# yewsiang/Transferable3D

Hardware: AMD Instinct MI355X
Metric: frustums/sec fwd+bwd (higher is better)
Workload: dtype f32

## Files before the change

transferable3d_amd/csrc/pointmlp.hip:

```cpp
#include "common.h"
#include "poolbwd_dev.h"
#include "rider_dev.h"

#include <cstdlib>
#include <mutex>
#include <type_traits>
#include <utility>
#include <unordered_map>

namespace {

constexpr int BK = 32;
constexpr int MIN_WAVES_PER_EU = 2;
constexpr int LDR = BK + 4;
constexpr int NT = 256;

__device__ __forceinline__ float4 f4zero() { return make_float4(0.f, 0.f, 0.f, 0.f); }

__device__ __forceinline__ unsigned keep_bits32(const float* __restrict__ rowmask, int base) {
  float4 m[8];
#pragma unroll
  for (int q = 0; q < 8; ++q) m[q] = *reinterpret_cast<const float4*>(rowmask + base + (q >> 2) * 32 + (q & 3) * 8);
  unsigned bits = 0u;
#pragma unroll
// ... 1285 lines not shown
    c.sh = *reinterpret_cast<const float4*>(reinterpret_cast<const char*>(shp + ucol) + lbytes);
    return c;
  }
  static constexpr bool HAS_CTAB = true;
  __device__ __forceinline__ int ctab_floats() const { return 2 * K; }
  __device__ __forceinline__ void ctab_fill(float* tab, int tid, int nthreads) const {
    const float* scp = s.scale != nullptr ? s.scale : t3d_ident_scale;
    const float* shp = s.scale != nullptr ? s.shift : t3d_ident_shift;
    for (int i = tid * 4; i < K; i += nthreads * 4) {
      *reinterpret_cast<float4*>(tab + i) = *reinterpret_cast<const float4*>(scp + i);
      *reinterpret_cast<float4*>(tab + K + i) = *reinterpret_cast<const float4*>(shp + i);
    }
  }
  __device__ __forceinline__ Coef ctab_coef(const float* tab, int col) const {
    Coef c;
    c.sc = *reinterpret_cast<const float4*>(tab + col);
    c.sh = *reinterpret_cast<const float4*>(tab + K + col);
    return c;
  }
  __device__ __forceinline__ Coef fetch_coef(int col) const {
    Coef c;
    c.sc = make_float4(1.f, 1.f, 1.f, 1.f);
    c.sh = f4zero();
    if (s.scale != nullptr) {
      c.sc = *reinterpret_cast<const float4*>(s.scale + col);
      c.sh = *reinterpret_cast<const float4*>(s.shift + col);
    }
    return c;
  }
  __device__ __forceinline__ Raw fetch(int row, int col) const {
    Raw r;
    r.x = *reinterpret_cast<const float4*>(s.x + (size_t)row * s.ldx + s.coff + col);
    return r;
  }
  __device__ __forceinline__ float4 xform(const Raw& r, const Coef& c, int, int) const {
    const float floor_ = s.relu ? 0.f : -INFINITY;
    return make_float4(fmaxf(fmaf(r.x.x, c.sc.x, c.sh.x), floor_), fmaxf(fmaf(r.x.y, c.sc.y, c.sh.y), floor_),
                       fmaxf(fmaf(r.x.z, c.sc.z, c.sh.z), floor_), fmaxf(fmaf(r.x.w, c.sc.w, c.sh.w), floor_));
  }
};

struct PathX3 {
  typedef float T;
  template <bool HAS_SUB, class XT> using Act = std::conditional_t<HAS_SUB, ActLoader<true>, ActLoaderE>;
  template <bool POOLED> using Dy = DyLoader<POOLED>;
  typedef WLoaderT<float> WL;
  typedef WLoaderT<float, true> WLX;
  static constexpr bool BF16 = false;
  static constexpr bool X3 = true;
  static constexpr int RED = BKX;
  template <int DIM, bool TYPE_R, class L, int PF, bool IS_A = false> using Stg = StagerX3<DIM, TYPE_R, L>;
};
template <class WL, bool FWD = true, class Args>
__device__ __forceinline__ WL make_wloader(const Args& p) {
  if constexpr (IsFrag<WL>::value) return WL{reinterpret_cast<const bf16_t*>(p.w_x3), (long)p.w_x3_stride, FWD ? p.N / 32 : p.K / 32};
  else return WL{p.w, p.N, p.K, p.N};
}
struct PathX3P : PathX3 {
  typedef WLoaderX3F WL;
  typedef WLoaderX3F WLX;
  template <int DIM, bool TYPE_R, class L, int PF, bool IS_A = false>
  using Stg = std::conditional_t<IsFrag<L>::value, StagerX3F<DIM, TYPE_R, L>, StagerX3<DIM, TYPE_R, L>>;
};
struct PathX3W : PathX3 {
  static constexpr int WAVES = 8;
  template <int DIM, bool TYPE_R, class L, int PF, bool IS_A = false> using Stg = StagerX3<DIM, TYPE_R, L, 2 * NT>;
};
struct PathX3WP : PathX3W {
  typedef WLoaderX3F WL;
  typedef WLoaderX3F WLX;
  template <int DIM, bool TYPE_R, class L, int PF, bool IS_A = false>
  using Stg = std::conditional_t<IsFrag<L>::value, StagerX3F<DIM, TYPE_R, L>, StagerX3<DIM, TYPE_R, L, 2 * NT>>;
};
template <class PR, class = void> struct WavesOf { static constexpr int value = 4; };
template <class PR> struct WavesOf<PR, typename std::enable_if<(PR::WAVES > 0)>::type> { static constexpr int value = PR::WAVES; };
template <class PR, int TM, int TN, class SA, class SB, class LA, class LB, bool AR, int DIMA, bool BR, int DIMB, bool SYM = false>
__device__ __forceinline__ void run_mainloop(SA& sa, SB& sb, const LA& la, const LB& lb, float* smem, int red_begin, int red_end,
                                             int a0, int b0, f32x16 (&acc)[TM][TN], int tid) {
  if constexpr (PR::X3) gemm_mainloop_x3<SYM, TM, TN, SA, SB, LA, LB, AR, DIMA, BR, DIMB>(sa, sb, la, lb, smem, red_begin, red_end, a0, b0, acc, tid);
  else if constexpr (PR::BF16) gemm_mainloop_h<TM, TN, SA, SB, LA, LB, AR, DIMA, BR, DIMB>(sa, sb, la, lb, smem, red_begin, red_end, a0, b0, acc, tid);
  else gemm_mainloop<TM, TN, SA, SB, LA, LB, AR, DIMA, BR, DIMB>(sa, sb, la, lb, smem, red_begin, red_end, a0, b0, acc, tid);
}

template <int BN, bool HAS_SUB, class PR = PathF32, class XT = float>
__device__ __forceinline__ void fwd_body(const t3d_pointmlp_fwd_args& p, float* smem, const int bid, const int nblk) {
  constexpr int BM = 128, TM = 2;
  constexpr int WN = WavesOf<PR>::value / 2, WCOLS = BN / WN, TN = WCOLS / 32;
  static_assert(TN == 1 || TN == 2, "a wave owns 32 or 64 columns");
  using LA = typename PR::template Act<HAS_SUB, XT>;
  using YT = typename PR::T;
  using WL = std::conditional_t<LA::EXACT, typename PR::WLX, typename PR::WL>;
  using SA = typename PR::template Stg<BM, true, LA, (PR::BF16 && BN == 128 && !Elem<XT>::BF16) ? 0 : 1, true>;
  using SB = typename PR::template Stg<BN, false, WL, 1>;

  const int tid = (int)threadIdx.x, lane = tid & 63, wid = tid >> 6;
  const int wm = wid / WN, wn = wid % WN;
  const int tiles_n = p.N / BN;
  const int lin = xcd_remap(bid, nblk);
  const int tile_m = lin / tiles_n, tile_n = lin % tiles_n;
  const int row0 = tile_m * BM, col0 = tile_n * BN;
  T3D_TRACE_MARK(0);

  LA la{p.a, p.K, p.rows_per_frustum};
  WL lb = make_wloader<WL>(p);
  SA sa; SB sb;
  sa.init(la, row0, tid);
  sb.init(lb, col0, tid);

  float addv[TN], addr[TN];
  {
    const int l31_ = lane & 31, b_ = row0 / p.rows_per_frustum;
#pragma unroll
    for (int tn = 0; tn < TN; ++tn) {
      const int col = col0 + wn * WCOLS + tn * 32 + l31_;
      addv[tn] = p.bias ? p.bias[col] : 0.f;
      addr[tn] = p.rowbias ? p.rowbias[(size_t)b_ * p.N + col] : 0.f;
    }
  }
  const bool has_rowbias = p.rowbias != nullptr;
  f32x16 acc[TM][TN];
  zero_acc<TM, TN>(acc);
  const int kred = (p.K + PR::RED - 1) / PR::RED * PR::RED;
  run_mainloop<PR, TM, TN, SA, SB, LA, WL, true, BM, false, BN>(sa, sb, la, lb, smem, 0, kred, wm * 64,
                                                                     wn * WCOLS, acc, tid);
  T3D_TRACE_MARK(1);

  const int l31 = lane & 31, h = lane >> 5;
  const int b = row0 / p.rows_per_frustum;
  const bool pool = p.pmax != nullptr;
  const bool store_y = p.y != nullptr;
  float* red = smem;
  constexpr int YLD = BN + 8;
  bf16_t* ytile = reinterpret_cast<bf16_t*>(smem + 12 * BN);
  float csum[TN], csq[TN], cmax[TN], cmin[TN];
  int amax[TN], amin[TN];
  unsigned keepbits = 0xffffffffu;
  if (pool && p.rowmask) {
    static_assert(TM == 2, "keep_bits32 covers two 32-row blocks");
    keepbits = keep_bits32(p.rowmask, row0 + wm * 64 + 4 * h);
  }
  const int rin_base = row0 - b * p.rows_per_frustum + wm * 64 + 4 * h;
  const unsigned n4 = (unsigned)p.N * 4u;
  char* const yb = reinterpret_cast<char*>(p.y);
  auto epi = [&](auto sy_tag, auto pl_tag) {
    constexpr bool SY = decltype(sy_tag)::value, PL = decltype(pl_tag)::value;
#pragma unroll
    for (int tn = 0; tn < TN; ++tn) {
      const int col = col0 + wn * WCOLS + tn * 32 + l31;
      const float add = has_rowbias ? addv[tn] + addr[tn] : addv[tn];
      float s = 0.f, ss = 0.f, mx = -INFINITY, mn = INFINITY;
      int ax = -1, an = -1;
      unsigned boff0 = ((unsigned)(row0 + wm * 64 + 4 * h) * (unsigned)p.N + (unsigned)col) * 4u;
      asm volatile("" : "+v"(boff0));
#pragma unroll
      for (int tm = 0; tm < TM; ++tm) {
#pragma unroll
        for (int r = 0; r < 16; ++r) {
          const float v = SY ? Elem<YT>::rnd(acc[tm][tn][r] + add) : acc[tm][tn][r] + add;
          if constexpr (SY) {
            if constexpr (Elem<YT>::BF16) {
              ytile[(wm * 64 + 4 * h + tm * 32 + (r & 3) + 8 * (r >> 2)) * YLD + wn * WCOLS + tn * 32 + l31] = (bf16_t)v;
            } else {
              *reinterpret_cast<float*>(yb + (boff0 + (unsigned)(tm * 32 + (r & 3) + 8 * (r >> 2)) * n4)) = v;
            }
          }
          s += v;
          ss = fmaf(v, v, ss);
          if constexpr (PL) {
            const bool keep = (keepbits >> (tm * 16 + r)) & 1u;
            const int rin = rin_base + tm * 32 + (r & 3) + 8 * (r >> 2);
            const bool up = keep & (v > mx), dn = keep & (v < mn);
            mx = up ? v : mx;
            ax = up ? rin : ax;
            mn = dn ? v : mn;
            an = dn ? rin : an;
          }
        }
      }
      s += __shfl_xor(s, 32, 64);
      ss += __shfl_xor(ss, 32, 64);
      if constexpr (PL) {
        const float omx = __shfl_xor(mx, 32, 64), omn = __shfl_xor(mn, 32, 64);
        const int oax = __shfl_xor(ax, 32, 64), oan = __shfl_xor(an, 32, 64);
        if (oax >= 0 && (omx > mx || ax < 0 || (omx == mx && oax < ax))) { mx = omx; ax = oax; }
        if (oan >= 0 && (omn < mn || an < 0 || (omn == mn && oan < an))) { mn = omn; an = oan; }
      }
      csum[tn] = s; csq[tn] = ss; cmax[tn] = mx; cmin[tn] = mn; amax[tn] = ax; amin[tn] = an;
    }
  };
  if (store_y) { if (pool) epi(std::true_type{}, std::true_type{}); else epi(std::true_type{}, std::false_type{}); }
  else { if (pool) epi(std::false_type{}, std::true_type{}); else epi(std::false_type{}, std::false_type{}); }
  __syncthreads();
  if (h == 0) {
#pragma unroll
    for (int tn = 0; tn < TN; ++tn) {
      const int c = wn * WCOLS + tn * 32 + l31;
      red[(0 * 2 + wm) * BN + c] = csum[tn];
      red[(1 * 2 + wm) * BN + c] = csq[tn];
      if (pool) {
        red[(2 * 2 + wm) * BN + c] = cmax[tn];
        red[(3 * 2 + wm) * BN + c] = cmin[tn];
        reinterpret_cast<int*>(red)[(4 * 2 + wm) * BN + c] = amax[tn];
        reinterpret_cast<int*>(red)[(5 * 2 + wm) * BN + c] = amin[tn];
      }
    }
  }
  __syncthreads();
  if (tid < BN) {
    const int c = tid;
    const size_t o = (size_t)tile_m * p.N + col0 + c;
    p.psum[o] = red[(0 * 2 + 0) * BN + c] + red[(0 * 2 + 1) * BN + c];
    p.psumsq[o] = red[(1 * 2 + 0) * BN + c] + red[(1 * 2 + 1) * BN + c];
    if (pool) {
      float mx = red[(2 * 2 + 0) * BN + c], mn = red[(3 * 2 + 0) * BN + c];
      int ax = reinterpret_cast<int*>(red)[(4 * 2 + 0) * BN + c], an = reinterpret_cast<int*>(red)[(5 * 2 + 0) * BN + c];
      const float mx1 = red[(2 * 2 + 1) * BN + c], mn1 = red[(3 * 2 + 1) * BN + c];
      const int ax1 = reinterpret_cast<int*>(red)[(4 * 2 + 1) * BN + c], an1 = reinterpret_cast<int*>(red)[(5 * 2 + 1) * BN + c];
      if (ax1 >= 0 && (ax < 0 || mx1 > mx)) { mx = mx1; ax = ax1; }
      if (an1 >= 0 && (an < 0 || mn1 < mn)) { mn = mn1; an = an1; }
      p.pmax[o] = mx; p.pmin[o] = mn; p.pamax[o] = ax; p.pamin[o] = an;
    }
  }
  if (store_y) {
    if constexpr (Elem<YT>::BF16) {
      constexpr int CPR = BN / 8;
      bf16_t* yg = reinterpret_cast<bf16_t*>(p.y);
#pragma unroll
      for (int i = 0; i < 128 * CPR / NT; ++i) {
        const int c = tid + NT * i, row = c / CPR, ch = c % CPR;
        const bf16x8 v = *reinterpret_cast<const bf16x8*>(ytile + row * YLD + ch * 8);
        *reinterpret_cast<bf16x8*>(yg + (size_t)(row0 + row) * p.N + col0 + ch * 8) = v;
      }
    }
  }
  T3D_TRACE_MARK(2);
}

template <int BN, bool HAS_SUB, class PR = PathF32, class XT = float>
__global__ __launch_bounds__(NT, MIN_WAVES_PER_EU) void k_pointmlp_fwd(const t3d_pointmlp_fwd_args p) {
  extern __shared__ __attribute__((aligned(16))) float smem[];
  fwd_body<BN, HAS_SUB, PR, XT>(p, smem, blockIdx.x, gridDim.x);
}

template <int BN, class PR>
__global__ __launch_bounds__(2 * NT) void k_pointmlp_fwd_w8(const t3d_pointmlp_fwd_args p, const int n_tiles) {
  extern __shared__ __attribute__((aligned(16))) float smem[];
  for (int b = blockIdx.x; b < n_tiles; b += gridDim.x) {
    int bb = b;
    asm volatile("" : "+s"(bb));
    fwd_body<BN, false, PR, float>(p, smem, bb, n_tiles);
    __syncthreads();
  }
}
template <int BN, class PR>
__global__ __launch_bounds__(2 * NT) void k_pointmlp_fwd_w8_r(const t3d_pointmlp_fwd_args p, const t3d_rider_set r, const int n_tiles) {
  extern __shared__ __attribute__((aligned(16))) float smem[];
  if ((int)blockIdx.x < r.n_wg) {
    if (threadIdx.x >= NT) return;
    run_riders(r, smem);
    return;
  }
  for (int b = blockIdx.x - r.n_wg; b < n_tiles; b += gridDim.x - r.n_wg) {
    int bb = b;
    asm volatile("" : "+s"(bb));
    fwd_body<BN, false, PR, float>(p, smem, bb, n_tiles);
    __syncthreads();
  }
}

template <int BN, bool HAS_SUB, class PR = PathF32>
__global__ __launch_bounds__(NT, MIN_WAVES_PER_EU) void k_pointmlp_fwd_r(const t3d_pointmlp_fwd_args p, const t3d_rider_set r) {
  extern __shared__ __attribute__((aligned(16))) float smem[];
  if ((int)blockIdx.x < r.n_wg) { run_riders(r, smem); return; }
  fwd_body<BN, HAS_SUB, PR, float>(p, smem, blockIdx.x - r.n_wg, gridDim.x - r.n_wg);
}

template <int BN, int KT>
__global__ __launch_bounds__(NT, MIN_WAVES_PER_EU) void k_pointmlp_fwd_res(const t3d_pointmlp_fwd_args p) {
  constexpr int TM = 2, TN = BN / 64, ST = BKH / 16;
  using LA = ActLoaderT<false, bf16_t>;
  using WL = WLoaderT<bf16_t, true>;
  using SA = StagerHSel<128, true, LA, KT>;
  using SB = StagerHSel<BN, false, WL, 1>;
  constexpr int A_ELEMS = SA::LDS_ELEMS, B_ELEMS = SB::LDS_ELEMS;
  static_assert((size_t)2 * B_ELEMS * 2 >= (size_t)12 * BN * 4 + (size_t)128 * (BN + 8) * 2, "the epilogue scratch aliases the weight ring");
  extern __shared__ __attribute__((aligned(16))) float smem[];
  bf16_t* panel = reinterpret_cast<bf16_t*>(smem);
  bf16_t* bst = panel + KT * A_ELEMS;

  const int tid0 = threadIdx.x;
  int tid = tid0, lane = tid & 63, wid = tid >> 6;
  int wm = wid >> 1, wn = wid & 1, l31 = lane & 31, h = lane >> 5;
  const bool pool = p.pmax != nullptr, store_y = p.y != nullptr;
  const int tiles_m = p.M / 128, G = gridDim.x;
  LA la{p.a, p.K, p.rows_per_frustum};
  SA sa;
  constexpr bool PREF = KT <= 2;
  auto fetch_panel = [&](int t_m) {
    sa.init(la, t_m * 128, tid);
    sa.template fetch_raw<0>(la, 0, tid);
    if constexpr (KT > 1) sa.template fetch_raw<1>(la, BKH, tid);
    if constexpr (KT > 2) { sa.template fetch_raw<2>(la, 2 * BKH, tid); sa.template fetch_raw<3>(la, 3 * BKH, tid); }
  };
  auto fetch_panel_coefs = [&]() {
    sa.template fetch_coefs<0>(la, 0, tid);
    if constexpr (KT > 1) sa.template fetch_coefs<1>(la, BKH, tid);
    if constexpr (KT > 2) { sa.template fetch_coefs<2>(la, 2 * BKH, tid); sa.template fetch_coefs<3>(la, 3 * BKH, tid); }
  };
  WL lb{p.w, p.N, p.K, p.N};
  SB sb;
  const int n_tiles = p.N / BN;
  float addv[TN], addr[TN];
  const bool has_rowbias = p.rowbias != nullptr;
  auto fetch_w0 = [&](int c0, int bb) {
    sb.init(lb, c0, tid);
    sb.template fetch<0>(lb, 0, tid);
#pragma unroll
    for (int tn = 0; tn < TN; ++tn) {
      const int col = c0 + wn * (BN / 2) + tn * 32 + l31;
      addv[tn] = p.bias ? p.bias[col] : 0.f;
      addr[tn] = has_rowbias ? p.rowbias[(size_t)bb * p.N + col] : 0.f;
    }
  };
  int tile_m = xcd_remap(blockIdx.x, G);
  T3D_TRACE_MARK8(0);
  if constexpr (PREF) { fetch_panel(tile_m); fetch_panel_coefs(); }
  fetch_w0(0, (tile_m * 128) / p.rows_per_frustum);
#pragma unroll 1
 for (; tile_m < tiles_m; tile_m += G) {
  const bool tr_first = tile_m < G;
  tid = tid0;
  asm volatile("" : "+v"(tid));
  lane = tid & 63; wid = tid >> 6; wm = wid >> 1; wn = wid & 1; l31 = lane & 31; h = lane >> 5;
  const int row0 = tile_m * 128;
  const int b = row0 / p.rows_per_frustum;
  if constexpr (!PREF) { fetch_panel(tile_m); fetch_panel_coefs(); }
  sa.template store<0>(la, panel, tid);
  if constexpr (KT > 1) sa.template store<1>(la, panel + A_ELEMS, tid);
  if constexpr (KT > 2) { sa.template store<2>(la, panel + 2 * A_ELEMS, tid); sa.template store<3>(la, panel + 3 * A_ELEMS, tid); }
  if (tr_first) T3D_TRACE_MARK8(1);
  unsigned keepbits = 0xffffffffu;
  if (pool && p.rowmask) {
    static_assert(TM == 2, "keep_bits32 covers two 32-row blocks");
    keepbits = keep_bits32(p.rowmask, row0 + wm * 64 + 4 * h);
  }
  const int rin_base = row0 - b * p.rows_per_frustum + wm * 64 + 4 * h;
  float* red = reinterpret_cast<float*>(bst);
  constexpr int YLD = BN + 8, CPR = BN / 8;
  bf16_t* ytile = reinterpret_cast<bf16_t*>(red + 12 * BN);
// ... 1911 lines not shown
                                                       const t3d_x3_frag_entry* __restrict__ tab, int n) {
  split_x3_frag_body(params, pf, pd, stride, tab, n, (int)blockIdx.x);
}

template <int N>
__global__ __launch_bounds__(NT) void k_step_head(const t3d_pointmlp_fwd_args p, const int n_fwd, const float* __restrict__ params,
                                                  bf16_t* __restrict__ pf, bf16_t* __restrict__ pd, const long stride,
                                                  const t3d_x3_frag_entry* __restrict__ tab, const int n, const int n_split, float* hyper,
                                                  const t3d_schedule sched) {
  __shared__ float red[2][NT / (N / 8)][N];
  const int b = blockIdx.x;
  if (b < n_fwd) pointmlp_fwd_tinyk_body<N, float>(p, red, b);
  else if (b < n_fwd + n_split) split_x3_frag_body(params, pf, pd, stride, tab, n, b - n_fwd);
  else if (threadIdx.x < 64) schedule_step_body(hyper, sched, threadIdx.x);
}
}
int t3d_x3_step_head(const t3d_pointmlp_fwd_args* a, const float* params, void* pf, void* pd, int64_t stride, const t3d_x3_frag_entry* tab, int n,
                     int n_blocks, float* hyper, const t3d_schedule* sched, hipStream_t s) {
  static_assert(NT == 256, "the three roles of k_step_head are 256-thread workgroups");
  const int n_fwd = a->M / 128;
  const dim3 grid(n_fwd + n_blocks + 1);
  if (a->N == 64) T3D_LAUNCH(k_step_head<64>, grid, dim3(NT), 0, s, *a, n_fwd, params, static_cast<bf16_t*>(pf), static_cast<bf16_t*>(pd), (long)stride, tab, n, n_blocks, hyper, *sched);
  else T3D_LAUNCH(k_step_head<128>, grid, dim3(NT), 0, s, *a, n_fwd, params, static_cast<bf16_t*>(pf), static_cast<bf16_t*>(pd), (long)stride, tab, n, n_blocks, hyper, *sched);
  T3D_CHECK_LAUNCH();
  return T3D_OK;
}
int t3d_x3_split_frag(const float* params, void* pf, void* pd, int64_t stride, const t3d_x3_frag_entry* tab, int n, int n_blocks, hipStream_t s) {
  T3D_LAUNCH(k_split_x3_frag, dim3(n_blocks), dim3(256), 0, s, params, static_cast<bf16_t*>(pf), static_cast<bf16_t*>(pd), (long)stride, tab, n);
  T3D_CHECK_LAUNCH();
  return T3D_OK;
}
int t3d_x3_split(const float* src, void* planes, int64_t n, int64_t plane_stride, hipStream_t s) {
  long blocks = (n + 1023) / 1024;
  if (blocks > 2048) blocks = 2048;
  T3D_LAUNCH(k_split_x3, dim3((unsigned)blocks), dim3(256), 0, s, src, static_cast<bf16_t*>(planes), (long)n, (long)plane_stride);
  T3D_CHECK_LAUNCH();
  return T3D_OK;
}

int t3d_x3_dgrad(const t3d_pointmlp_dgrad_args* a, bool wide, hipStream_t s) {
  const int tiles_m = a->M / 128;
  if (a->w_x3 && (a->K % 32 != 0 || a->N % 16 != 0 || a->w_x3_stride < (int64_t)a->K * a->N)) return T3D_ERR_SHAPE;
  if (a->w_x3 && a->N <= X3_CTAB_MAX_CH) {
    if (wide) launch_lds(k_pointmlp_dgrad<128, false, PathX3P>, dim3(tiles_m * (a->K / 128)), lds_dgrad_x3(128), s, *a);
    else launch_lds(k_pointmlp_dgrad<64, false, PathX3P>, dim3(tiles_m * (a->K / 64)), lds_dgrad_x3(64), s, *a);
  } else if (wide) launch_lds(k_pointmlp_dgrad<128, false, PathX3>, dim3(tiles_m * (a->K / 128)), lds_dgrad_x3(128), s, *a);
  else launch_lds(k_pointmlp_dgrad<64, false, PathX3>, dim3(tiles_m * (a->K / 64)), lds_dgrad_x3(64), s, *a);
  T3D_CHECK_LAUNCH();
  return T3D_OK;
}

int t3d_x3_wgrad(const t3d_pointmlp_wgrad_args* a, int tk, int tn, int n_blocks, hipStream_t s) {
  const dim3 grid(n_blocks);
#define T3D_WGX(TK, TN_) launch_lds(k_pointmlp_wgrad<TK, TN_, false, false, PathX3, float>, grid, lds_wgrad_x3(TK, TN_), s, *a)
  if (tk == 128 && tn == 128) T3D_WGX(128, 128);
  else if (tk == 128) T3D_WGX(128, 64);
  else if (tn == 128) T3D_WGX(64, 128);
  else T3D_WGX(64, 64);
#undef T3D_WGX
  T3D_CHECK_LAUNCH();
  return T3D_OK;
}

int t3d_x3_gram(const t3d_pointmlp_gram_args* a, int tk, int n_blocks, hipStream_t s) {
  if (tk != 64) return T3D_ERR_ARG;
  launch_lds(k_pointmlp_gram<64, 64, PathX3>, dim3(n_blocks), lds_wgrad_x3(64, 64), s, *a);
  T3D_CHECK_LAUNCH();
  return T3D_OK;
}

int t3d_x3_dgrad_gram(const t3d_pointmlp_dgrad_gram_args* a, bool wide, hipStream_t s) {
  const int tiles_m = a->M / 128;
  if (wide) launch_lds(k_pointmlp_dgrad_gram<128, PathX3>, dim3(tiles_m * (a->K / 128)), lds_fwd_x3(128), s, *a);
  else launch_lds(k_pointmlp_dgrad_gram<64, PathX3>, dim3(tiles_m * (a->K / 64)), lds_fwd_x3(64), s, *a);
  T3D_CHECK_LAUNCH();
  return T3D_OK;
}

int t3d_x3_fwd(const t3d_pointmlp_fwd_args* a, const t3d_rider_set* r, hipStream_t s) {
  const int tiles_m = a->M / 128, nr = r ? r->n_wg : 0;
  const bool pre = a->w_x3 != nullptr && a->K <= X3_CTAB_MAX_CH;
  if (pre && (a->N % 32 != 0 || a->K % 16 != 0 || a->w_x3_stride < (int64_t)a->K * a->N)) return T3D_ERR_SHAPE;
  const int w8 = []() { const char* e_ = getenv("T3D_X3_W8"); return e_ ? atoi(e_) : 1; }();
  if (w8 && a->N % 256 == 0 && (w8 == 2 || (long)tiles_m * (a->N / 256) >= 512)) {
    const int n_tiles = tiles_m * (a->N / 256);
    const dim3 grid((n_tiles > T3D_FAIR_CUS ? T3D_FAIR_CUS : n_tiles) + nr);
    const size_t lds = lds_with(lds_fwd_x3(256), r);
    if (r && pre) {
      auto kern = k_pointmlp_fwd_w8_r<256, PathX3WP>;
      allow_lds(reinterpret_cast<const void*>(kern), lds);
      T3D_LAUNCH(kern, grid, dim3(2 * NT), lds, s, *a, *r, n_tiles);
    } else if (r) {
      auto kern = k_pointmlp_fwd_w8_r<256, PathX3W>;
      allow_lds(reinterpret_cast<const void*>(kern), lds);
      T3D_LAUNCH(kern, grid, dim3(2 * NT), lds, s, *a, *r, n_tiles);
    } else if (pre) {
      auto kern = k_pointmlp_fwd_w8<256, PathX3WP>;
      allow_lds(reinterpret_cast<const void*>(kern), lds);
      T3D_LAUNCH(kern, grid, dim3(2 * NT), lds, s, *a, n_tiles);
    } else {
      auto kern = k_pointmlp_fwd_w8<256, PathX3W>;
      allow_lds(reinterpret_cast<const void*>(kern), lds);
      T3D_LAUNCH(kern, grid, dim3(2 * NT), lds, s, *a, n_tiles);
    }
    T3D_CHECK_LAUNCH();
    return T3D_OK;
  }
  if (a->N % 128 == 0 && (long)tiles_m * (a->N / 128) >= 512) {
    const dim3 grid(tiles_m * (a->N / 128) + nr);
    if (r && pre) launch_lds_r(k_pointmlp_fwd_r<128, false, PathX3P>, grid, lds_with(lds_fwd_x3(128), r), s, *a, *r);
    else if (r) launch_lds_r(k_pointmlp_fwd_r<128, false, PathX3>, grid, lds_with(lds_fwd_x3(128), r), s, *a, *r);
    else if (pre) launch_lds(k_pointmlp_fwd<128, false, PathX3P, float>, grid, lds_fwd_x3(128), s, *a);
    else launch_lds(k_pointmlp_fwd<128, false, PathX3, float>, grid, lds_fwd_x3(128), s, *a);
  } else {
    const dim3 grid(tiles_m * (a->N / 64) + nr);
    if (r && pre) launch_lds_r(k_pointmlp_fwd_r<64, false, PathX3P>, grid, lds_with(lds_fwd_x3(64), r), s, *a, *r);
    else if (r) launch_lds_r(k_pointmlp_fwd_r<64, false, PathX3>, grid, lds_with(lds_fwd_x3(64), r), s, *a, *r);
    else if (pre) launch_lds(k_pointmlp_fwd<64, false, PathX3P, float>, grid, lds_fwd_x3(64), s, *a);
    else launch_lds(k_pointmlp_fwd<64, false, PathX3, float>, grid, lds_fwd_x3(64), s, *a);
  }
  T3D_CHECK_LAUNCH();
  return T3D_OK;
}

int t3d_x3_bwd(const t3d_pointmlp_dgrad_args* d, const t3d_pointmlp_wgrad_args* w, const t3d_rider_set* r, int tk, int tn, bool wide,
               int n_w, int n_d, hipStream_t s) {
  if (d->w_x3 && (d->K % 32 != 0 || d->N % 16 != 0 || d->w_x3_stride < (int64_t)d->K * d->N)) return T3D_ERR_SHAPE;
  const dim3 grid(n_w + n_d + (r ? r->n_wg : 0));
#define T3D_BWDX_P(DBN, TK, TN_, PR_)                                                             \
  do {                                                                                             \
    const size_t lds = lds_max(lds_dgrad_x3(DBN), lds_wgrad_x3(TK, TN_));                          \
    if (r) {                                                                                       \
      auto kern = k_pointmlp_bwd_r<DBN, TK, TN_, PR_>;                                             \
      allow_lds(reinterpret_cast<const void*>(kern), lds_with(lds, r));                            \
      T3D_LAUNCH(kern, grid, dim3(NT), lds_with(lds, r), s, *d, *w, n_w, *r);                      \
    } else {                                                                                       \
      auto kern = k_pointmlp_bwd<DBN, TK, TN_, PR_>;                                               \
      allow_lds(reinterpret_cast<const void*>(kern), lds);                                         \
      T3D_LAUNCH(kern, grid, dim3(NT), lds, s, *d, *w, n_w);                                       \
    }                                                                                              \
  } while (0)
#define T3D_BWDX(DBN, TK, TN_) do { if (d->w_x3 && d->N <= X3_CTAB_MAX_CH) T3D_BWDX_P(DBN, TK, TN_, PathX3P); else T3D_BWDX_P(DBN, TK, TN_, PathX3); } while (0)
#define T3D_BWDX_W(DBN)                                  \
  do {                                                   \
    if (tk == 128 && tn == 128) T3D_BWDX(DBN, 128, 128); \
    else if (tk == 128) T3D_BWDX(DBN, 128, 64);          \
    else if (tn == 128) T3D_BWDX(DBN, 64, 128);          \
    else T3D_BWDX(DBN, 64, 64);                          \
  } while (0)
  if (wide) T3D_BWDX_W(128);
  else T3D_BWDX_W(64);
#undef T3D_BWDX_W
#undef T3D_BWDX
#undef T3D_BWDX_P
  T3D_CHECK_LAUNCH();
  return T3D_OK;
}

int t3d_x3_stage1(const t3d_pointmlp_gram_args* g, const t3d_act_colsum_args* c, const t3d_pool_bwd_prep_args* q, const t3d_rider_set* r,
                  int gt, int n_gram, int n_colsum, int n_prep, size_t lds_other, hipStream_t s) {
  const dim3 grid(n_gram + n_colsum + n_prep + (r ? r->n_wg : 0));
  const size_t lds = lds_with(lds_max(lds_wgrad_x3(gt, gt), lds_other), r);
#define T3D_ST1X(GT_)                                                                  \
  do {                                                                                 \
    if (r) {                                                                           \
      auto kern = k_pool_bwd_stage1_r<GT_, PathX3>;                                    \
      allow_lds(reinterpret_cast<const void*>(kern), lds);                             \
// ... 795 lines not shown
```

Measured before the change: 27690.

## Add activation-resident x3 forward kernel that sweeps all column tiles per row tile

Adds a new forward kernel for K=64/128 that loads and splits a 128-row activation tile into three bf16 planes in LDS once, then loops over every 256-column weight tile. This reuses the activation tile instead of re-staging it for each column tile. The kernel software-pipelines fragment loads behind the MFMAs and overlaps the cross-wave partial-stat reduction with the next tile's compute. It does this by splitting the waves into a writer half and a storer half with double-buffered reduction slots. The epilogue is factored into reusable helpers, and the new path is taken by default when the weight-fragment x3 path applies with no riders. In exchange the grid is smaller (one block per row tile) and LDS use is larger.

Measured after the change: 27850, median of 6. Within noise of the previous version (+0.6%).

```diff
diff --git a/transferable3d_amd/csrc/pointmlp.hip b/transferable3d_amd/csrc/pointmlp.hip
--- a/transferable3d_amd/csrc/pointmlp.hip
+++ b/transferable3d_amd/csrc/pointmlp.hip
@@ -1391,63 +1391,21 @@
   else gemm_mainloop<TM, TN, SA, SB, LA, LB, AR, DIMA, BR, DIMB>(sa, sb, la, lb, smem, red_begin, red_end, a0, b0, acc, tid);
 }
 
-template <int BN, bool HAS_SUB, class PR = PathF32, class XT = float>
-__device__ __forceinline__ void fwd_body(const t3d_pointmlp_fwd_args& p, float* smem, const int bid, const int nblk) {
-  constexpr int BM = 128, TM = 2;
-  constexpr int WN = WavesOf<PR>::value / 2, WCOLS = BN / WN, TN = WCOLS / 32;
-  static_assert(TN == 1 || TN == 2, "a wave owns 32 or 64 columns");
-  using LA = typename PR::template Act<HAS_SUB, XT>;
-  using YT = typename PR::T;
-  using WL = std::conditional_t<LA::EXACT, typename PR::WLX, typename PR::WL>;
-  using SA = typename PR::template Stg<BM, true, LA, (PR::BF16 && BN == 128 && !Elem<XT>::BF16) ? 0 : 1, true>;
-  using SB = typename PR::template Stg<BN, false, WL, 1>;
-
-  const int tid = (int)threadIdx.x, lane = tid & 63, wid = tid >> 6;
+template <int TN> struct FwdColPart { float csum[TN], csq[TN], cmax[TN], cmin[TN]; int amax[TN], amin[TN]; };
+
+template <int BN, int TN, int WN, class YT>
+__device__ __forceinline__ void fwd_epi_lane(const t3d_pointmlp_fwd_args& p, bf16_t* ytile, const f32x16 (&acc)[2][TN], const float (&addv)[TN],
+                                             const float (&addr)[TN], const bool has_rowbias, const unsigned keepbits, const int tile_m,
+                                             const int col0, const int tid, FwdColPart<TN>& q) {
+  constexpr int TM = 2, WCOLS = BN / WN;
+  const int lane = tid & 63, wid = tid >> 6;
   const int wm = wid / WN, wn = wid % WN;
-  const int tiles_n = p.N / BN;
-  const int lin = xcd_remap(bid, nblk);
-  const int tile_m = lin / tiles_n, tile_n = lin % tiles_n;
-  const int row0 = tile_m * BM, col0 = tile_n * BN;
-  T3D_TRACE_MARK(0);
-
-  LA la{p.a, p.K, p.rows_per_frustum};
-  WL lb = make_wloader<WL>(p);
-  SA sa; SB sb;
-  sa.init(la, row0, tid);
-  sb.init(lb, col0, tid);
-
-  float addv[TN], addr[TN];
-  {
-    const int l31_ = lane & 31, b_ = row0 / p.rows_per_frustum;
-#pragma unroll
-    for (int tn = 0; tn < TN; ++tn) {
-      const int col = col0 + wn * WCOLS + tn * 32 + l31_;
-      addv[tn] = p.bias ? p.bias[col] : 0.f;
-      addr[tn] = p.rowbias ? p.rowbias[(size_t)b_ * p.N + col] : 0.f;
-    }
-  }
-  const bool has_rowbias = p.rowbias != nullptr;
-  f32x16 acc[TM][TN];
-  zero_acc<TM, TN>(acc);
-  const int kred = (p.K + PR::RED - 1) / PR::RED * PR::RED;
-  run_mainloop<PR, TM, TN, SA, SB, LA, WL, true, BM, false, BN>(sa, sb, la, lb, smem, 0, kred, wm * 64,
-                                                                     wn * WCOLS, acc, tid);
-  T3D_TRACE_MARK(1);
-
+  const int row0 = tile_m * 128;
+  const int b = row0 / p.rows_per_frustum;
   const int l31 = lane & 31, h = lane >> 5;
-  const int b = row0 / p.rows_per_frustum;
   const bool pool = p.pmax != nullptr;
   const bool store_y = p.y != nullptr;
-  float* red = smem;
   constexpr int YLD = BN + 8;
-  bf16_t* ytile = reinterpret_cast<bf16_t*>(smem + 12 * BN);
-  float csum[TN], csq[TN], cmax[TN], cmin[TN];
-  int amax[TN], amin[TN];
-  unsigned keepbits = 0xffffffffu;
-  if (pool && p.rowmask) {
-    static_assert(TM == 2, "keep_bits32 covers two 32-row blocks");
-    keepbits = keep_bits32(p.rowmask, row0 + wm * 64 + 4 * h);
-  }
   const int rin_base = row0 - b * p.rows_per_frustum + wm * 64 + 4 * h;
   const unsigned n4 = (unsigned)p.N * 4u;
   char* const yb = reinterpret_cast<char*>(p.y);
@@ -1494,41 +1452,67 @@
         if (oax >= 0 && (omx > mx || ax < 0 || (omx == mx && oax < ax))) { mx = omx; ax = oax; }
         if (oan >= 0 && (omn < mn || an < 0 || (omn == mn && oan < an))) { mn = omn; an = oan; }
       }
-      csum[tn] = s; csq[tn] = ss; cmax[tn] = mx; cmin[tn] = mn; amax[tn] = ax; amin[tn] = an;
+      q.csum[tn] = s; q.csq[tn] = ss; q.cmax[tn] = mx; q.cmin[tn] = mn; q.amax[tn] = ax; q.amin[tn] = an;
     }
   };
   if (store_y) { if (pool) epi(std::true_type{}, std::true_type{}); else epi(std::true_type{}, std::false_type{}); }
   else { if (pool) epi(std::false_type{}, std::true_type{}); else epi(std::false_type{}, std::false_type{}); }
+}
+
+__device__ __forceinline__ void fwd_epi_store(const t3d_pointmlp_fwd_args& p, const bool pool, const size_t o, const float s0, const float s1,
+                                              const float q0, const float q1, float mx, const float mx1, float mn, const float mn1, int ax,
+                                              const int ax1, int an, const int an1) {
+  p.psum[o] = s0 + s1;
+  p.psumsq[o] = q0 + q1;
+  if (pool) {
+    if (ax1 >= 0 && (ax < 0 || mx1 > mx)) { mx = mx1; ax = ax1; }
+    if (an1 >= 0 && (an < 0 || mn1 < mn)) { mn = mn1; an = an1; }
+    p.pmax[o] = mx; p.pmin[o] = mn; p.pamax[o] = ax; p.pamin[o] = an;
+  }
+}
+
+template <int BN, int TN, int WN, class YT>
+__device__ __forceinline__ void fwd_epilogue(const t3d_pointmlp_fwd_args& p, float* red, const f32x16 (&acc)[2][TN], const float (&addv)[TN],
+                                             const float (&addr)[TN], const bool has_rowbias, const unsigned keepbits, const int tile_m,
+                                             const int col0, const int tid) {
+  constexpr int WCOLS = BN / WN;
+  const int lane = tid & 63, wid = tid >> 6;
+  const int wm = wid / WN, wn = wid % WN;
+  const int row0 = tile_m * 128;
+  const int l31 = lane & 31, h = lane >> 5;
+  const bool pool = p.pmax != nullptr;
+  const bool store_y = p.y != nullptr;
+  constexpr int YLD = BN + 8;
+  bf16_t* ytile = reinterpret_cast<bf16_t*>(red + 12 * BN);
+  FwdColPart<TN> q;
+  fwd_epi_lane<BN, TN, WN, YT>(p, ytile, acc, addv, addr, has_rowbias, keepbits, tile_m, col0, tid, q);
   __syncthreads();
   if (h == 0) {
 #pragma unroll
     for (int tn = 0; tn < TN; ++tn) {
       const int c = wn * WCOLS + tn * 32 + l31;
-      red[(0 * 2 + wm) * BN + c] = csum[tn];
-      red[(1 * 2 + wm) * BN + c] = csq[tn];
+      red[(0 * 2 + wm) * BN + c] = q.csum[tn];
+      red[(1 * 2 + wm) * BN + c] = q.csq[tn];
       if (pool) {
-        red[(2 * 2 + wm) * BN + c] = cmax[tn];
-        red[(3 * 2 + wm) * BN + c] = cmin[tn];
-        reinterpret_cast<int*>(red)[(4 * 2 + wm) * BN + c] = amax[tn];
-        reinterpret_cast<int*>(red)[(5 * 2 + wm) * BN + c] = amin[tn];
+        red[(2 * 2 + wm) * BN + c] = q.cmax[tn];
+        red[(3 * 2 + wm) * BN + c] = q.cmin[tn];
+        reinterpret_cast<int*>(red)[(4 * 2 + wm) * BN + c] = q.amax[tn];
+        reinterpret_cast<int*>(red)[(5 * 2 + wm) * BN + c] = q.amin[tn];
       }
     }
   }
   __syncthreads();
   if (tid < BN) {
     const int c = tid;
-    const size_t o = (size_t)tile_m * p.N + col0 + c;
-    p.psum[o] = red[(0 * 2 + 0) * BN + c] + red[(0 * 2 + 1) * BN + c];
-    p.psumsq[o] = red[(1 * 2 + 0) * BN + c] + red[(1 * 2 + 1) * BN + c];
+    const int* redi = reinterpret_cast<const int*>(red);
+    float mx = 0.f, mx1 = 0.f, mn = 0.f, mn1 = 0.f;
+    int ax = -1, ax1 = -1, an = -1, an1 = -1;
     if (pool) {
-      float mx = red[(2 * 2 + 0) * BN + c], mn = red[(3 * 2 + 0) * BN + c];
-      int ax = reinterpret_cast<int*>(red)[(4 * 2 + 0) * BN + c], an = reinterpret_cast<int*>(red)[(5 * 2 + 0) * BN + c];
-      const float mx1 = red[(2 * 2 + 1) * BN + c], mn1 = red[(3 * 2 + 1) * BN + c];
-      const int ax1 = reinterpret_cast<int*>(red)[(4 * 2 + 1) * BN + c], an1 = reinterpret_cast<int*>(red)[(5 * 2 + 1) * BN + c];
-      if (ax1 >= 0 && (ax < 0 || mx1 > mx)) { mx = mx1; ax = ax1; }
-      if (an1 >= 0 && (an < 0 || mn1 < mn)) { mn = mn1; an = an1; }
-      p.pmax[o] = mx; p.pmin[o] = mn; p.pamax[o] = ax; p.pamin[o] = an;
-    }
+      mx = red[(2 * 2 + 0) * BN + c]; mx1 = red[(2 * 2 + 1) * BN + c]; mn = red[(3 * 2 + 0) * BN + c]; mn1 = red[(3 * 2 + 1) * BN + c];
+      ax = redi[(4 * 2 + 0) * BN + c]; ax1 = redi[(4 * 2 + 1) * BN + c]; an = redi[(5 * 2 + 0) * BN + c]; an1 = redi[(5 * 2 + 1) * BN + c];
+    }
+    fwd_epi_store(p, pool, (size_t)tile_m * p.N + col0 + c, red[(0 * 2 + 0) * BN + c], red[(0 * 2 + 1) * BN + c], red[(1 * 2 + 0) * BN + c],
+                  red[(1 * 2 + 1) * BN + c], mx, mx1, mn, mn1, ax, ax1, an, an1);
   }
   if (store_y) {
     if constexpr (Elem<YT>::BF16) {
@@ -1542,6 +1526,57 @@
       }
     }
   }
+}
+
+template <int BN, bool HAS_SUB, class PR = PathF32, class XT = float>
+__device__ __forceinline__ void fwd_body(const t3d_pointmlp_fwd_args& p, float* smem, const int bid, const int nblk) {
+  constexpr int BM = 128, TM = 2;
+  constexpr int WN = WavesOf<PR>::value / 2, WCOLS = BN / WN, TN = WCOLS / 32;
+  static_assert(TN == 1 || TN == 2, "a wave owns 32 or 64 columns");
+  using LA = typename PR::template Act<HAS_SUB, XT>;
+  using YT = typename PR::T;
+  using WL = std::conditional_t<LA::EXACT, typename PR::WLX, typename PR::WL>;
+  using SA = typename PR::template Stg<BM, true, LA, (PR::BF16 && BN == 128 && !Elem<XT>::BF16) ? 0 : 1, true>;
+  using SB = typename PR::template Stg<BN, false, WL, 1>;
+
+  const int tid = (int)threadIdx.x, lane = tid & 63, wid = tid >> 6;
+  const int wm = wid / WN, wn = wid % WN;
+  const int tiles_n = p.N / BN;
+  const int lin = xcd_remap(bid, nblk);
+  const int tile_m = lin / tiles_n, tile_n = lin % tiles_n;
+  const int row0 = tile_m * BM, col0 = tile_n * BN;
+  T3D_TRACE_MARK(0);
+
+  LA la{p.a, p.K, p.rows_per_frustum};
+  WL lb = make_wloader<WL>(p);
+  SA sa; SB sb;
+  sa.init(la, row0, tid);
+  sb.init(lb, col0, tid);
+
+  float addv[TN], addr[TN];
+  {
+    const int l31_ = lane & 31, b_ = row0 / p.rows_per_frustum;
+#pragma unroll
+    for (int tn = 0; tn < TN; ++tn) {
+      const int col = col0 + wn * WCOLS + tn * 32 + l31_;
+      addv[tn] = p.bias ? p.bias[col] : 0.f;
+      addr[tn] = p.rowbias ? p.rowbias[(size_t)b_ * p.N + col] : 0.f;
+    }
+  }
+  const bool has_rowbias = p.rowbias != nullptr;
+  f32x16 acc[TM][TN];
+  zero_acc<TM, TN>(acc);
+  const int kred = (p.K + PR::RED - 1) / PR::RED * PR::RED;
+  run_mainloop<PR, TM, TN, SA, SB, LA, WL, true, BM, false, BN>(sa, sb, la, lb, smem, 0, kred, wm * 64,
+                                                                     wn * WCOLS, acc, tid);
+  T3D_TRACE_MARK(1);
+
+  unsigned keepbits = 0xffffffffu;
+  if (p.pmax != nullptr && p.rowmask) {
+    static_assert(TM == 2, "keep_bits32 covers two 32-row blocks");
+    keepbits = keep_bits32(p.rowmask, row0 + wm * 64 + 4 * (lane >> 5));
+  }
+  fwd_epilogue<BN, TN, WN, YT>(p, smem, acc, addv, addr, has_rowbias, keepbits, tile_m, col0, tid);
   T3D_TRACE_MARK(2);
 }
 
@@ -1574,6 +1609,170 @@
     asm volatile("" : "+s"(bb));
     fwd_body<BN, false, PR, float>(p, smem, bb, n_tiles);
     __syncthreads();
+  }
+}
+
+template <int TM, int TN, class WL>
+__device__ __forceinline__ void x3_iter_res(const FragsX3<TM, TN>& fc, FragsX3<TM, TN>& fn, const bf16_t* an, const WL& lb, const int cn,
+                                            const int red_next, const int lane, f32x16 (&acc)[TM][TN]) {
+  constexpr int NM = 6 * TM * TN, PLANE = 128 * LDRX;
+  static_assert(3 * (TM + TN) * 2 <= NM, "one fragment request behind every second MFMA");
+  static_for<NM>([&](auto ic) {
+    constexpr int i = decltype(ic)::value;
+    constexpr int p = i / (TM * TN), tm = (i / TN) % TM, tn = i % TN;
+    constexpr int pa = p == 0 ? 2 : (p == 2 || p == 3) ? 1 : 0;
+    constexpr int pb = p == 1 ? 2 : (p == 2 || p == 4) ? 1 : 0;
+    acc[tm][tn] = __builtin_amdgcn_mfma_f32_32x32x16_bf16(fc.a[pa][tm], fc.b[pb][tn], acc[tm][tn], 0, 0, 0);
+    T3D_PIN1(acc[tm][tn]);
+    __builtin_amdgcn_sched_barrier(0);
+    if constexpr (i % 2 == 0 && i / 2 < 3 * (TM + TN)) {
+      constexpr int k = i / 2;
+      asm volatile("" ::: "memory");
+      if constexpr (k < 3 * TN) {
+        constexpr int o = k / TN, x = k % TN, pl = o == 0 ? 0 : o == 1 ? 2 : 1;
+        fn.b[pl][x] = lb.gfrag(pl, cn + x * 32, red_next, lane);
+      } else {
+        constexpr int j = k - 3 * TN, o = j / TM, x = j % TM, pl = o == 0 ? 2 : o == 1 ? 0 : 1;
+        fn.a[pl][x] = *reinterpret_cast<const bf16x8*>(an + pl * PLANE + x * 32 * LDRX);
+      }
+      asm volatile("" ::: "memory");
+    }
+    __builtin_amdgcn_sched_barrier(0);
+  });
+}
+
+constexpr int ARES_BN = 256;
+constexpr size_t lds_fwd_ares(int k) { return (size_t)(k / BKX) * 3 * 128 * LDRX * 2 + (size_t)12 * ARES_BN * sizeof(float); }
+
+template <int K, class PR>
+__global__ __launch_bounds__(2 * NT) void k_pointmlp_fwd_ares(const t3d_pointmlp_fwd_args p) {
+  constexpr int BN = ARES_BN, TM = 2, TN = 2, WN = 4, WCOLS = BN / WN, KT = K / BKX;
+  static_assert(WavesOf<PR>::value == 2 * WN && IsFrag<typename PR::WLX>::value, "eight waves, weights in fragment order");
+  static_assert(KT >= 2 && KT % 2 == 0, "the k loop takes two k-tiles per pass");
+  static_assert(BN == WN * 64 && TN == 2, "thread tid of the upper half stores column tid: its wave holds it");
+  using LA = ActLoaderE;
+  using WL = typename PR::WLX;
+  using SA = StagerX3<128, true, LA, 2 * NT>;
+  static_assert(SA::NV == 1, "one piece per thread and k-tile");
+  constexpr int PLANE = SA::PLANE, IMG = SA::LDS_ELEMS;
+  extern __shared__ __attribute__((aligned(16))) float smem[];
+  float* const red = smem + KT * IMG / 2;
+  const int tiles_m = p.M / 128, n_ct = p.N / BN;
+  const LA la{p.a, p.K, p.rows_per_frustum};
+  const WL lb = make_wloader<WL>(p);
+  const bool has_rowbias = p.rowbias != nullptr;
+#pragma unroll 1
+  for (int bt = blockIdx.x; bt < tiles_m; bt += gridDim.x) {
+    int bb = bt, tid = (int)threadIdx.x;
+    asm volatile("" : "+s"(bb));
+    asm volatile("" : "+v"(tid));
+    const int lane = tid & 63, wid = tid >> 6, wm = wid / WN, wn = wid % WN;
+    const int tile_m = xcd_remap(bb, tiles_m), row0 = tile_m * 128;
+    {
+      int li, ri;
+      SA::coords(tid, 0, li, ri);
+      typename LA::Raw raw[KT];
+      typename LA::Coef cf[KT];
+#pragma unroll
+      for (int t = 0; t < KT; ++t) raw[t] = la.fetch(row0 + li, t * BKX + ri);
+#pragma unroll
+      for (int t = 0; t < KT; ++t) cf[t] = la.fetch_coef(t * BKX + ri);
+#pragma unroll
+      for (int t = 0; t < KT; ++t) {
+        bf16x4 h, m, lo;
+        split3(la.xform(raw[t], cf[t], row0 + li, t * BKX + ri), h, m, lo);
+        bf16_t* dst = reinterpret_cast<bf16_t*>(smem) + t * IMG + x3_r_off(li, ri);
+        *reinterpret_cast<bf16x4*>(dst) = h;
+        *reinterpret_cast<bf16x4*>(dst + PLANE) = m;
+        *reinterpret_cast<bf16x4*>(dst + 2 * PLANE) = lo;
+      }
+    }
+    unsigned keepbits = 0xffffffffu;
+    if (p.pmax != nullptr && p.rowmask) keepbits = keep_bits32(p.rowmask, row0 + wm * 64 + 4 * (lane >> 5));
+    const int b0 = wn * WCOLS;
+    const bf16_t* const a_lane = reinterpret_cast<const bf16_t*>(smem) + x3_r_off(wm * 64 + (lane & 31), 8 * (lane >> 5));
+    const bool lower = __builtin_amdgcn_readfirstlane(wid) >= WN;
+    const bool pool = p.pmax != nullptr;
+    float own_f[4];
+    int own_i[2];
+    auto res_store = [&](const int ct_) {
+      const float* rr = red + (ct_ & 1) * 6 * BN;
+      const int c = tid;
+      float mx1 = 0.f, mn1 = 0.f;
+      int ax1 = -1, an1 = -1;
+      if (pool) { mx1 = rr[2 * BN + c]; mn1 = rr[3 * BN + c]; ax1 = reinterpret_cast<const int*>(rr)[4 * BN + c]; an1 = reinterpret_cast<const int*>(rr)[5 * BN + c]; }
+      fwd_epi_store(p, pool, (size_t)tile_m * p.N + ct_ * BN + c, own_f[0], rr[0 * BN + c], own_f[1], rr[1 * BN + c], own_f[2], mx1, own_f[3], mn1,
+                    own_i[0], ax1, own_i[1], an1);
+    };
+    FragsX3<TM, TN> f0, f1;
+#pragma unroll
+    for (int pl = 0; pl < 3; ++pl)
+#pragma unroll
+      for (int tn = 0; tn < TN; ++tn) f0.b[pl][tn] = lb.gfrag(pl, b0 + tn * 32, 0, lane);
+    __syncthreads();
+#pragma unroll
+    for (int pl = 0; pl < 3; ++pl)
+#pragma unroll
+      for (int tm = 0; tm < TM; ++tm) f0.a[pl][tm] = *reinterpret_cast<const bf16x8*>(a_lane + pl * PLANE + tm * 32 * LDRX);
+#pragma unroll 1
+    for (int ct = 0; ct < n_ct; ++ct) {
+      const int col0 = ct * BN;
+      const int coln = (ct + 1 < n_ct ? ct + 1 : 0) * BN;
+      float addv[TN], addr[TN];
+      {
+        const int b_ = row0 / p.rows_per_frustum;
+#pragma unroll
+        for (int tn = 0; tn < TN; ++tn) {
+          const int col = col0 + b0 + tn * 32 + (lane & 31);
+          addv[tn] = p.bias ? p.bias[col] : 0.f;
+          addr[tn] = has_rowbias ? p.rowbias[(size_t)b_ * p.N + col] : 0.f;
+        }
+      }
+      f32x16 acc[TM][TN];
+      zero_acc<TM, TN>(acc);
+#pragma unroll 1
+      for (int t = 0; t < KT; t += 2) {
+        x3_iter_res<TM, TN, WL>(f0, f1, a_lane + (t + 1) * IMG, lb, col0 + b0, (t + 1) * BKX, lane, acc);
+        const bool wrap = t + 2 == KT;
+        const int tn_ = wrap ? 0 : t + 2;
+        x3_iter_res<TM, TN, WL>(f1, f0, a_lane + tn_ * IMG, lb, (wrap ? coln : col0) + b0, tn_ * BKX, lane, acc);
+      }
+      float* const redw = red + (ct & 1) * 6 * BN;
+      if (!lower && ct > 0) {
+        __syncthreads();
+        res_store(ct - 1);
+      }
+      FwdColPart<TN> q;
+      fwd_epi_lane<BN, TN, WN, float>(p, nullptr, acc, addv, addr, has_rowbias, keepbits, tile_m, col0, tid, q);
+      if (lower) {
+        if (lane < 32) {
+#pragma unroll
+          for (int tn = 0; tn < TN; ++tn) {
+            const int c = b0 + tn * 32 + lane;
+            redw[0 * BN + c] = q.csum[tn];
+            redw[1 * BN + c] = q.csq[tn];
+            if (pool) {
+              redw[2 * BN + c] = q.cmax[tn];
+              redw[3 * BN + c] = q.cmin[tn];
+              reinterpret_cast<int*>(redw)[4 * BN + c] = q.amax[tn];
+              reinterpret_cast<int*>(redw)[5 * BN + c] = q.amin[tn];
+            }
+          }
+        }
+        __syncthreads();
+      } else {
+        const bool hi = lane >= 32;
+        const float s1 = __shfl_xor(q.csum[1], 32, 64), q1 = __shfl_xor(q.csq[1], 32, 64);
+        const float x1 = __shfl_xor(q.cmax[1], 32, 64), n1 = __shfl_xor(q.cmin[1], 32, 64);
+        const int ax1 = __shfl_xor(q.amax[1], 32, 64), an1 = __shfl_xor(q.amin[1], 32, 64);
+        own_f[0] = hi ? s1 : q.csum[0]; own_f[1] = hi ? q1 : q.csq[0]; own_f[2] = hi ? x1 : q.cmax[0]; own_f[3] = hi ? n1 : q.cmin[0];
+        own_i[0] = hi ? ax1 : q.amax[0]; own_i[1] = hi ? an1 : q.amin[0];
+      }
+    }
+    if (!lower) {
+      __syncthreads();
+      res_store(n_ct - 1);
+    }
   }
 }
 
@@ -3651,7 +3850,25 @@
   const bool pre = a->w_x3 != nullptr && a->K <= X3_CTAB_MAX_CH;
   if (pre && (a->N % 32 != 0 || a->K % 16 != 0 || a->w_x3_stride < (int64_t)a->K * a->N)) return T3D_ERR_SHAPE;
   const int w8 = []() { const char* e_ = getenv("T3D_X3_W8"); return e_ ? atoi(e_) : 1; }();
-  if (w8 && a->N % 256 == 0 && (w8 == 2 || (long)tiles_m * (a->N / 256) >= 512)) {
+  const bool take_w8 = w8 && a->N % 256 == 0 && (w8 == 2 || (long)tiles_m * (a->N / 256) >= 512);
+  const int ares = []() { const char* e_ = getenv("T3D_X3_ARES"); return e_ ? atoi(e_) : 1; }();
+  if (ares && (ares == 2 || take_w8) && pre && !r && (a->K == 64 || a->K == 128) && a->N % ARES_BN == 0 && a->N >= 2 * ARES_BN) {
+    const size_t lds = lds_fwd_ares(a->K);
+    if (lds > 160 * 1024) return T3D_ERR_SHAPE;
+    const dim3 grid(tiles_m > T3D_FAIR_CUS ? T3D_FAIR_CUS : tiles_m);
+    if (a->K == 128) {
+      auto kern = k_pointmlp_fwd_ares<128, PathX3WP>;
+      allow_lds(reinterpret_cast<const void*>(kern), lds);
+      T3D_LAUNCH(kern, grid, dim3(2 * NT), lds, s, *a);
+    } else {
+      auto kern = k_pointmlp_fwd_ares<64, PathX3WP>;
+      allow_lds(reinterpret_cast<const void*>(kern), lds);
+      T3D_LAUNCH(kern, grid, dim3(2 * NT), lds, s, *a);
+    }
+    T3D_CHECK_LAUNCH();
+    return T3D_OK;
+  }
+  if (take_w8) {
     const int n_tiles = tiles_m * (a->N / 256);
     const dim3 grid((n_tiles > T3D_FAIR_CUS ? T3D_FAIR_CUS : n_tiles) + nr);
     const size_t lds = lds_with(lds_fwd_x3(256), r);
```
